# kanyu369/ADNM-UNet

Measured on AMD Instinct MI355X. Metric: sequences/sec training ADNM-UNet 5->20x128x128, higher is better.
Workload: dtype bf16; 1 GPU; ADNM-UNet create_ADNMUNet(5,20,6) 128x128 full training step (fwd + enRainfallLoss + bwd + clip_grad_norm_ + AdamW), recipe parameters, synthetic radar frames in HBM; per_gpu_batch=4, global_batch=4, frames=5->20, parallelism=single, launch=hipGraph replay

## Files before the change

### adnm-unet_amd/csrc/conv3.hip

```cpp
#include "adnm_common.h"

namespace {

using f32x4 = adnm_f32x4;
constexpr int kBlock = 256, kWaves = 4;
constexpr int CK = 16, CKP = CK + 4;
constexpr int MB = 2;
constexpr int kTilePix = kWaves * MB * 16;

struct Geo {
  int TW, RB, TH;
  int tiles_x, tiles_y, VR;
};
inline Geo make_geo(int64_t B, int64_t H, int64_t W) {
  Geo g;
  g.TW = (W == 4 || W == 8) ? (int)W : 16;
  g.RB = 16 / g.TW;
  g.TH = kWaves * MB * g.RB;
  g.VR = (int)(B * (H + 1));
  g.tiles_x = (int)adnm_cdiv(W, g.TW);
  g.tiles_y = (int)adnm_cdiv(g.VR, g.TH);
  return g;
}

// ... 222 lines not shown
  }
  if (rec_a) adnm_amax_commit(&a.q->amax_a, amax_a);
  if (rec_b) adnm_amax_commit(&a.q->amax_b, amax_b);
  if (PREC == ADNM_MFMA_FP8) {
    const float inv = 1.0f / (q_sa * q_sb);
#pragma unroll
    for (int nb = 0; nb < NB; ++nb)
#pragma unroll
      for (int mb = 0; mb < MB; ++mb) acc[nb][mb] = acc[nb][mb] * inv;
  }
  conv3_epilogue<NB, ACT_OUT>(a, acc, wave, kk, dyj, dxj, x0, v0, n0);
}

template <int NB, int ACT_IN, int ACT_OUT>
__global__ __launch_bounds__(kBlock) void conv3_bf16_kernel(ConvArgs a) {
  extern __shared__ __attribute__((aligned(16))) float smem[];
  constexpr int CN = 2 * CK;
  float amax_a = 0.f, amax_b = 0.f;
  bool rec_a = false, rec_b = false;
  if (a.q) {
    const bool rec = a.q->record != 0.f;
    rec_a = rec && blockIdx.y == 0, rec_b = rec && blockIdx.x == 0;
  }
  const int TWp = a.TW + 2;
  float* sIn = smem;
  float* sW = smem + (a.TH + 2) * TWp * CKP;
  const int wave = threadIdx.x >> 6, lane = threadIdx.x & 63, j = lane & 15, kk = lane >> 4;
  const int tx = blockIdx.x % a.tiles_x, ty = blockIdx.x / a.tiles_x;
  const int x0 = tx * a.TW, v0 = ty * a.TH, n0 = blockIdx.y * NB * 16;
  const int dyj = j / a.TW, dxj = j - dyj * a.TW;
  int base[MB];
#pragma unroll
  for (int mb = 0; mb < MB; ++mb) base[mb] = (((wave * MB + mb) * a.RB + dyj) * TWp + dxj) * CKP + 4 * kk;
  f32x4 acc[NB][MB];
#pragma unroll
  for (int nb = 0; nb < NB; ++nb)
#pragma unroll
    for (int mb = 0; mb < MB; ++mb) acc[nb][mb] = f32x4{0.f, 0.f, 0.f, 0.f};
  const int kbeg = blockIdx.z * a.chunks_per_split * CK;
  const int kend = kbeg + a.chunks_per_split * CK < a.K ? kbeg + a.chunks_per_split * CK : a.K;
  constexpr int kItIn = 4;
  constexpr int kItW = (9 * NB * 64 + kBlock - 1) / kBlock;
  const int PT = (a.TH + 2) * TWp;
  float rin[kItIn][8], rw[kItW][8];
  auto load_chunk = [&](int c0) {
#pragma unroll
    for (int u = 0; u < kItIn; ++u) {
      const int it = threadIdx.x + u * kBlock;
      const int pix = it >> 2, q = it & 3, r = pix / TWp, cc = pix - r * TWp, ch = c0 + 8 * q;
      const int64_t p = it < PT * 4 ? pixel_of(v0 - 1 + r, x0 - 1 + cc, a.B, a.H, a.W, a.VR) : -1;
      float v[8] = {0.f, 0.f, 0.f, 0.f, 0.f, 0.f, 0.f, 0.f};
      if (p >= 0 && ch < kend) {
        if (a.vec_in && ch + 7 < kend) {
          const float4 t0 = *reinterpret_cast<const float4*>(a.in + p * a.ldin + ch), t1 = *reinterpret_cast<const float4*>(a.in + p * a.ldin + ch + 4);
          v[0] = t0.x; v[1] = t0.y; v[2] = t0.z; v[3] = t0.w; v[4] = t1.x; v[5] = t1.y; v[6] = t1.z; v[7] = t1.w;
          if (ACT_IN != ADNM_ACT_NONE) {
            const float4 g0 = *reinterpret_cast<const float4*>(a.in2 + p * a.ldin2 + ch), g1 = *reinterpret_cast<const float4*>(a.in2 + p * a.ldin2 + ch + 4);
            v[0] *= act_grad<ACT_IN>(g0.x); v[1] *= act_grad<ACT_IN>(g0.y); v[2] *= act_grad<ACT_IN>(g0.z); v[3] *= act_grad<ACT_IN>(g0.w);
            v[4] *= act_grad<ACT_IN>(g1.x); v[5] *= act_grad<ACT_IN>(g1.y); v[6] *= act_grad<ACT_IN>(g1.z); v[7] *= act_grad<ACT_IN>(g1.w);
          }
        } else {
#pragma unroll
          for (int e = 0; e < 8; ++e)
            if (ch + e < kend) {
              v[e] = a.in[p * a.ldin + ch + e];
              if (ACT_IN != ADNM_ACT_NONE) v[e] *= act_grad<ACT_IN>(a.in2[p * a.ldin2 + ch + e]);
            }
        }
      }
#pragma unroll
      for (int e = 0; e < 8; ++e) rin[u][e] = v[e];
    }
#pragma unroll
    for (int u = 0; u < kItW; ++u) {
      const int it = threadIdx.x + u * kBlock;
      const int kq = it & 3, nl = (it >> 2) % (NB * 16), tap = it / (NB * 64);
      const int n = n0 + nl, k0 = c0 + 8 * kq;
      float v[8] = {0.f, 0.f, 0.f, 0.f, 0.f, 0.f, 0.f, 0.f};
      if (it < 9 * NB * 64 && n < a.N && k0 < kend) {
        const float* wp = a.w + (int64_t)n * a.sn + (int64_t)(a.flip ? 8 - tap : tap) * a.st + (int64_t)k0 * a.sk;
        if (a.vec_w && k0 + 7 < kend) {
          const float4 t0 = *reinterpret_cast<const float4*>(wp), t1 = *reinterpret_cast<const float4*>(wp + 4);
          v[0] = t0.x; v[1] = t0.y; v[2] = t0.z; v[3] = t0.w; v[4] = t1.x; v[5] = t1.y; v[6] = t1.z; v[7] = t1.w;
        } else {
#pragma unroll
          for (int e = 0; e < 8; ++e)
            if (k0 + e < kend) v[e] = wp[(int64_t)e * a.sk];
        }
      }
#pragma unroll
      for (int e = 0; e < 8; ++e) rw[u][e] = v[e];
    }
  };
  auto store_chunk = [&]() {
#pragma unroll
    for (int u = 0; u < kItIn; ++u) {
      const int it = threadIdx.x + u * kBlock;
      if (it >= PT * 4) break;
      if (rec_a) amax_a = adnm_amax4(adnm_amax4(amax_a, rin[u][0], rin[u][1], rin[u][2], rin[u][3]), rin[u][4], rin[u][5], rin[u][6], rin[u][7]);
      *reinterpret_cast<adnm_bf16x8*>(sIn + (it >> 2) * CKP + 4 * (it & 3)) = adnm_pack_bf16x8(rin[u]);
    }
#pragma unroll
    for (int u = 0; u < kItW; ++u) {
      const int it = threadIdx.x + u * kBlock;
      if (it >= 9 * NB * 64) break;
      const int kq = it & 3, nl = (it >> 2) % (NB * 16), tap = it / (NB * 64);
      if (rec_b) amax_b = adnm_amax4(adnm_amax4(amax_b, rw[u][0], rw[u][1], rw[u][2], rw[u][3]), rw[u][4], rw[u][5], rw[u][6], rw[u][7]);
      *reinterpret_cast<adnm_bf16x8*>(sW + (tap * NB * 16 + nl) * CKP + 4 * kq) = adnm_pack_bf16x8(rw[u]);
    }
  };
  if (kbeg < kend) load_chunk(kbeg);
  for (int c0 = kbeg; c0 < kend; c0 += CN) {
    __syncthreads();
    store_chunk();
    __syncthreads();
    if (c0 + CN < kend) load_chunk(c0 + CN);
#pragma unroll
    for (int tap = 0; tap < 9; ++tap) {
      const int toff = ((tap / 3) * TWp + (tap % 3)) * CKP;
      adnm_bf16x8 fw[NB], fx[MB];
#pragma unroll
      for (int nb = 0; nb < NB; ++nb) fw[nb] = *reinterpret_cast<const adnm_bf16x8*>(sW + (tap * NB * 16 + nb * 16 + j) * CKP + 4 * kk);
#pragma unroll
      for (int mb = 0; mb < MB; ++mb) fx[mb] = *reinterpret_cast<const adnm_bf16x8*>(sIn + base[mb] + toff);
#pragma unroll
      for (int nb = 0; nb < NB; ++nb)
#pragma unroll
        for (int mb = 0; mb < MB; ++mb) acc[nb][mb] = __builtin_amdgcn_mfma_f32_16x16x32_bf16(fw[nb], fx[mb], acc[nb][mb], 0, 0, 0);
    }
  }
  if (rec_a) adnm_amax_commit(&a.q->amax_a, amax_a);
  if (rec_b) adnm_amax_commit(&a.q->amax_b, amax_b);
  conv3_epilogue<NB, ACT_OUT>(a, acc, wave, kk, dyj, dxj, x0, v0, n0);
}

template <int ACT_OUT>
__global__ __launch_bounds__(256) void conv3_join_kernel(const float* __restrict__ part, int nsplit, int64_t M, int N, const float* __restrict__ bias,
                                                         float* __restrict__ out, int64_t ldo, float* __restrict__ pre, int64_t ldpre) {
  const int nq = N >> 2;
  const int64_t i = (int64_t)blockIdx.x * 256 + threadIdx.x;
  if (i >= M * nq) return;
  const int64_t p = i / nq;
  const int n = (int)(i - p * nq) * 4;
  float4 s = *reinterpret_cast<const float4*>(part + p * N + n);
  for (int z = 1; z < nsplit; ++z) {
    const float4 t = *reinterpret_cast<const float4*>(part + ((int64_t)z * M + p) * N + n);
    s.x += t.x; s.y += t.y; s.z += t.z; s.w += t.w;
  }
  if (bias) { s.x += bias[n]; s.y += bias[n + 1]; s.z += bias[n + 2]; s.w += bias[n + 3]; }
  if (pre) *reinterpret_cast<float4*>(pre + p * ldpre + n) = s;
  *reinterpret_cast<float4*>(out + p * ldo + n) = make_float4(act_fwd<ACT_OUT>(s.x), act_fwd<ACT_OUT>(s.y), act_fwd<ACT_OUT>(s.z), act_fwd<ACT_OUT>(s.w));
}

struct WgArgs {
  const float* dout; int64_t lddo;
  const float* pre;  int64_t ldpre;
  const float* in;   int64_t ldin;
  float* part; int64_t rowlen;
  int want_bias;
  int B, H, W, K, N, ntiles;
  int TW, RB, TH, VR, tiles_x;
  int vec_in, vec_do;
};

template <int NB, int ACT, int PREC>
__global__ __launch_bounds__(kBlock) void conv3_wgrad_kernel(WgArgs a) {
  constexpr int DP = NB * 16 + 16;
  extern __shared__ __attribute__((aligned(16))) float smem[];
  const int TWp = a.TW + 2;
  float* sIn = smem;
  float* sD = smem + (a.TH + 2) * TWp * CKP;
  const int wave = threadIdx.x >> 6, lane = threadIdx.x & 63, j = lane & 15, kk = lane >> 4;
  const int c0 = blockIdx.y * CK, n0 = blockIdx.z * NB * 16;
  f32x4 acc[9][NB];
#pragma unroll
  for (int t = 0; t < 9; ++t)
#pragma unroll
    for (int nb = 0; nb < NB; ++nb) acc[t][nb] = f32x4{0.f, 0.f, 0.f, 0.f};
  float bsum = 0.f;
  constexpr int kItIn = 4, kItD = (kTilePix * NB * 4 + kBlock - 1) / kBlock;
  const int PT = (a.TH + 2) * TWp;
  float rin[kItIn][4], rd[kItD][4];
  auto load_tile = [&](int tile) {
    const int tx = tile % a.tiles_x, ty = tile / a.tiles_x, x0 = tx * a.TW, v0 = ty * a.TH;
#pragma unroll
    for (int u = 0; u < kItIn; ++u) {
      const int it = threadIdx.x + u * kBlock;
      const int pix = it >> 2, q = it & 3, r = pix / TWp, cc = pix - r * TWp, ch = c0 + 4 * q;
      const int64_t p = it < PT * 4 ? pixel_of(v0 - 1 + r, x0 - 1 + cc, a.B, a.H, a.W, a.VR) : -1;
      float v[4] = {0.f, 0.f, 0.f, 0.f};
      if (p >= 0 && ch < a.K) {
        if (a.vec_in && ch + 3 < a.K) {
          const float4 t = *reinterpret_cast<const float4*>(a.in + p * a.ldin + ch);
          v[0] = t.x; v[1] = t.y; v[2] = t.z; v[3] = t.w;
        } else {
#pragma unroll
          for (int e = 0; e < 4; ++e)
            if (ch + e < a.K) v[e] = a.in[p * a.ldin + ch + e];
        }
      }
#pragma unroll
      for (int e = 0; e < 4; ++e) rin[u][e] = v[e];
    }
#pragma unroll
    for (int u = 0; u < kItD; ++u) {
      const int it = threadIdx.x + u * kBlock;
      const int pxl = it / (NB * 4), q = it - pxl * (NB * 4), n = n0 + 4 * q;
      const int pb = pxl >> 4, jj = pxl & 15, dy_ = jj / a.TW, dx_ = jj - dy_ * a.TW;
      const int64_t p = it < kTilePix * NB * 4 ? pixel_of(v0 + pb * a.RB + dy_, x0 + dx_, a.B, a.H, a.W, a.VR) : -1;
      float v[4] = {0.f, 0.f, 0.f, 0.f};
      if (p >= 0 && n < a.N) {
        if (a.vec_do && n + 3 < a.N) {
          const float4 t = *reinterpret_cast<const float4*>(a.dout + p * a.lddo + n);
          v[0] = t.x; v[1] = t.y; v[2] = t.z; v[3] = t.w;
          if (ACT != ADNM_ACT_NONE) {
            const float4 g = *reinterpret_cast<const float4*>(a.pre + p * a.ldpre + n);
            v[0] *= act_grad<ACT>(g.x); v[1] *= act_grad<ACT>(g.y); v[2] *= act_grad<ACT>(g.z); v[3] *= act_grad<ACT>(g.w);
          }
        } else {
#pragma unroll
          for (int e = 0; e < 4; ++e)
            if (n + e < a.N) {
              v[e] = a.dout[p * a.lddo + n + e];
              if (ACT != ADNM_ACT_NONE) v[e] *= act_grad<ACT>(a.pre[p * a.ldpre + n + e]);
            }
        }
      }
#pragma unroll
      for (int e = 0; e < 4; ++e) rd[u][e] = v[e];
    }
  };
  auto store_tile = [&]() {
#pragma unroll
    for (int u = 0; u < kItIn; ++u) {
      const int it = threadIdx.x + u * kBlock;
      if (it >= PT * 4) break;
      *reinterpret_cast<float4*>(sIn + (it >> 2) * CKP + 4 * (it & 3)) = make_float4(rin[u][0], rin[u][1], rin[u][2], rin[u][3]);
    }
#pragma unroll
    for (int u = 0; u < kItD; ++u) {
      const int it = threadIdx.x + u * kBlock;
      if (it >= kTilePix * NB * 4) break;
      const int pxl = it / (NB * 4), q = it - pxl * (NB * 4);
      *reinterpret_cast<float4*>(sD + pxl * DP + 4 * q) = make_float4(rd[u][0], rd[u][1], rd[u][2], rd[u][3]);
    }
  };
  if ((int)blockIdx.x < a.ntiles) load_tile(blockIdx.x);
  for (int tile = blockIdx.x; tile < a.ntiles; tile += gridDim.x) {
    __syncthreads();
    store_tile();
    __syncthreads();
    if (tile + (int)gridDim.x < a.ntiles) load_tile(tile + gridDim.x);
    static_assert(MB == 2, "the weight-gradient step pairs the wave's two pixel blocks");
    float av[NB][2][4];
    const float* bp[2][4];
#pragma unroll
    for (int pbw = 0; pbw < MB; ++pbw) {
      const int pb = wave * MB + pbw;
#pragma unroll
      for (int e = 0; e < 4; ++e) {
        const int jj = 4 * kk + e, pxl = pb * 16 + jj, dy_ = jj / a.TW, dx_ = jj - dy_ * a.TW;
#pragma unroll
        for (int nb = 0; nb < NB; ++nb) av[nb][pbw][e] = sD[pxl * DP + nb * 16 + j];
        bp[pbw][e] = sIn + ((pb * a.RB + dy_) * TWp + dx_) * CKP + j;
      }
    }
    AdnmFrag<PREC> fa[NB];
#pragma unroll
    for (int nb = 0; nb < NB; ++nb) fa[nb] = adnm_make_frag<PREC, false>(av[nb][0], av[nb][1], 1.f);
#pragma unroll
    for (int tap = 0; tap < 9; ++tap) {
      const int toff = ((tap / 3) * TWp + (tap % 3)) * CKP;
      const float b0[4] = {bp[0][0][toff], bp[0][1][toff], bp[0][2][toff], bp[0][3][toff]};
      const float b1[4] = {bp[1][0][toff], bp[1][1][toff], bp[1][2][toff], bp[1][3][toff]};
      const AdnmFrag<PREC> fb = adnm_make_frag<PREC, false>(b0, b1, 1.f);
#pragma unroll
      for (int nb = 0; nb < NB; ++nb) acc[tap][nb] = adnm_mma<PREC, false, false>(fa[nb], fb, acc[tap][nb]);
    }
    if (a.want_bias && blockIdx.y == 0 && lane < NB * 16) {
#pragma unroll 8
      for (int p = 0; p < MB * 16; ++p) bsum += sD[(wave * MB * 16 + p) * DP + lane];
    }
  }
  __syncthreads();
  float* red = smem;
  constexpr int kPer = 9 * NB * 4;
#pragma unroll
  for (int tap = 0; tap < 9; ++tap)
#pragma unroll
    for (int nb = 0; nb < NB; ++nb)
#pragma unroll
      for (int r = 0; r < 4; ++r) red[(wave * (kPer + 1) + (tap * NB + nb) * 4 + r) * 64 + lane] = acc[tap][nb][r];
  red[(wave * (kPer + 1) + kPer) * 64 + lane] = bsum;
  __syncthreads();
  float* dst = a.part + (int64_t)blockIdx.x * a.rowlen;
  for (int e = threadIdx.x; e < (kPer + 1) * 64; e += kBlock) {
    const float v = (red[e] + red[(kPer + 1) * 64 + e]) + (red[2 * (kPer + 1) * 64 + e] + red[3 * (kPer + 1) * 64 + e]);
    const int slot = e >> 6, ln = e & 63;
    if (slot == kPer) {
      if (a.want_bias && blockIdx.y == 0 && ln < NB * 16 && n0 + ln < a.N) dst[(int64_t)a.N * 9 * a.K + n0 + ln] = v;
      continue;
    }
    const int r = slot & 3, nb = (slot >> 2) % NB, tap = slot / (4 * NB);
    const int n = n0 + nb * 16 + (ln >> 4) * 4 + r, k = c0 + (ln & 15);
    if (n < a.N && k < a.K) dst[((int64_t)n * 9 + tap) * a.K + k] = v;
  }
}

inline bool al16(const void* p) { return ((uintptr_t)p & 15) == 0; }

int check_shape(const char* who, int64_t B, int64_t H, int64_t W, int64_t K, int64_t N) {
  ADNM_REQUIRE(B > 0 && H > 0 && W > 0 && K > 0 && N > 0, "%s: empty shape", who);
  ADNM_REQUIRE(B * (H + 1) < (1ll << 30) && B * H * W < (1ll << 31) && K <= 65536 && N <= 65536, "%s: shape too large", who);
  return ADNM_OK;
}

struct Split {
  int nb, ngroups, nsplit, cps;
};
inline Split plan_split(const Geo& g, int64_t K, int64_t N) {
  Split s;
  s.nb = N > 32 ? 4 : (N > 16 ? 2 : 1);
  s.ngroups = (int)adnm_cdiv(N, s.nb * 16);
  const int nchunks = (int)adnm_cdiv(K, CK);
  const int64_t blocks = (int64_t)g.tiles_x * g.tiles_y * s.ngroups;
  int want = 1;
  if (blocks < 256 && nchunks >= 4 && N % 4 == 0) {
    want = (int)adnm_cdiv(512, blocks);
    if (want > nchunks / 2) want = nchunks / 2;
    if (want > 16) want = 16;
    if (want < 1) want = 1;
  }
  s.cps = (int)adnm_cdiv(nchunks, want);
  if (want > 1 && (s.cps & 1)) ++s.cps;
  s.nsplit = (int)adnm_cdiv(nchunks, s.cps);
  return s;
}

template <int ACT_IN, int ACT_OUT>
int launch_conv(const ConvArgs& a, const Geo& g, const Split& s, int prec, hipStream_t st, const char* prof, double bytes) {
  const size_t smem = sizeof(float) * ((size_t)(g.TH + 2) * (g.TW + 2) * CKP + (size_t)9 * s.nb * 16 * CKP);
  const dim3 grid((unsigned)(g.tiles_x * g.tiles_y), (unsigned)s.ngroups, (unsigned)s.nsplit);
  ADNM_PROF(prof, st, bytes);
#define CV(PRECV, BF8V)                                                                                  \
  do {                                                                                                   \
    if (s.nb == 4) conv3_kernel<4, ACT_IN, ACT_OUT, PRECV, BF8V><<<grid, kBlock, smem, st>>>(a);         \
    else if (s.nb == 2) conv3_kernel<2, ACT_IN, ACT_OUT, PRECV, BF8V><<<grid, kBlock, smem, st>>>(a);    \
    else conv3_kernel<1, ACT_IN, ACT_OUT, PRECV, BF8V><<<grid, kBlock, smem, st>>>(a);                   \
  } while (0)
  static const bool fp32_images = getenv("ADNM_CONV3_FP32_IMAGES") && atoi(getenv("ADNM_CONV3_FP32_IMAGES")) != 0;
  if (prec == ADNM_MFMA_BF16 && fp32_images) CV(ADNM_MFMA_BF16, false);
  else if (prec == ADNM_MFMA_BF16) {
    if (s.nb == 4) conv3_bf16_kernel<4, ACT_IN, ACT_OUT><<<grid, kBlock, smem, st>>>(a);
    else if (s.nb == 2) conv3_bf16_kernel<2, ACT_IN, ACT_OUT><<<grid, kBlock, smem, st>>>(a);
    else conv3_bf16_kernel<1, ACT_IN, ACT_OUT><<<grid, kBlock, smem, st>>>(a);
  } else if (prec == ADNM_MFMA_FP8) CV(ADNM_MFMA_FP8, false);
  else if (prec == ADNM_MFMA_FP8_GRAD) CV(ADNM_MFMA_FP8, true);
  else CV(ADNM_MFMA_F32, false);
#undef CV
  return ADNM_OK;
}

void fill_geo(ConvArgs& a, const Geo& g) { a.TW = g.TW, a.RB = g.RB, a.TH = g.TH, a.VR = g.VR, a.tiles_x = g.tiles_x; }

}

extern "C" int64_t adnm_conv3_ws_bytes(int64_t B, int64_t H, int64_t W, int64_t K, int64_t N) {
  if (B <= 0 || H <= 0 || W <= 0 || K <= 0 || N <= 0) return 0;
  const Geo g = make_geo(B, H, W);
  const Split s = plan_split(g, K, N);
  return s.nsplit > 1 ? (int64_t)s.nsplit * B * H * W * N * (int64_t)sizeof(float) : 16;
}

extern "C" int adnm_conv3_fwd(const float* in, int64_t ldin, const float* w, int64_t ws_n, int64_t ws_tap, int64_t ws_k, const float* bias,
                              float* out, int64_t ldo, float* pre, int64_t ldpre, void* ws, int64_t ws_bytes, int64_t B, int64_t H, int64_t W,
                              int64_t K, int64_t N, int act, int prec, float* q, adnm_stream_t stream) {
  if (int rc = check_shape("conv3_fwd", B, H, W, K, N)) return rc;
  ADNM_REQUIRE(in && w && out, "conv3_fwd: null pointer");
  ADNM_REQUIRE(prec >= ADNM_MFMA_F32 && prec <= ADNM_MFMA_FP8, "conv3_fwd: bad prec %d", prec);
  ADNM_REQUIRE(prec != ADNM_MFMA_FP8 || q, "conv3_fwd: the fp8 mode needs a quantisation record");
  ADNM_REQUIRE(ldin >= K && ldo >= N && (!pre || ldpre >= N), "conv3_fwd: row strides smaller than the rows");
  ADNM_REQUIRE(act == ADNM_ACT_NONE || act == ADNM_ACT_GELU, "conv3_fwd: activation %d not in {none, gelu}", act);
  const Geo g = make_geo(B, H, W);
  const Split s = plan_split(g, K, N);
  if (s.nsplit > 1 && (!ws || ws_bytes < adnm_conv3_ws_bytes(B, H, W, K, N))) {
    adnm_set_error("conv3_fwd: workspace %lld < %lld bytes", (long long)ws_bytes, (long long)adnm_conv3_ws_bytes(B, H, W, K, N));
    return ADNM_EWORKSPACE;
  }
  ConvArgs a{};
  a.in = in, a.ldin = ldin, a.in2 = nullptr, a.ldin2 = 0;
  a.w = w, a.sn = ws_n, a.st = ws_tap, a.sk = ws_k, a.flip = 0;
  a.bias = bias, a.out = out, a.ldo = ldo, a.pre = pre, a.ldpre = ldpre, a.part = (float*)ws;
  a.B = (int)B, a.H = (int)H, a.W = (int)W, a.K = (int)K, a.N = (int)N, a.nsplit = s.nsplit, a.chunks_per_split = s.cps;
  fill_geo(a, g);
  a.vec_in = al16(in) && ldin % 4 == 0 && K % 4 == 0;
  a.vec_w = ws_k == 1 && al16(w) && ws_n % 4 == 0 && ws_tap % 4 == 0 && K % 4 == 0;
  a.vec_out = al16(out) && ldo % 4 == 0 && N % 4 == 0 && (!pre || (al16(pre) && ldpre % 4 == 0));
  a.q = reinterpret_cast<AdnmQuant*>(q);
  hipStream_t st = (hipStream_t)stream;
  const double bytes = 4.0 * ((double)B * H * W * (K + N * (pre ? 2 : 1)) + 9.0 * K * N);
  if (act == ADNM_ACT_GELU && s.nsplit == 1) launch_conv<ADNM_ACT_NONE, ADNM_ACT_GELU>(a, g, s, prec, st, "conv3_fwd", bytes);
  else launch_conv<ADNM_ACT_NONE, ADNM_ACT_NONE>(a, g, s, prec, st, "conv3_fwd", bytes);
  ADNM_CHECK_LAUNCH("conv3_fwd");
  if (s.nsplit > 1) {
    const int64_t M = B * H * W, nthreads = M * (N / 4);
    ADNM_PROF("conv3_join", st, 4.0 * M * N * (s.nsplit + 1 + (pre ? 1 : 0)));
    if (act == ADNM_ACT_GELU)
      conv3_join_kernel<ADNM_ACT_GELU><<<(unsigned)adnm_cdiv(nthreads, 256), 256, 0, st>>>((const float*)ws, s.nsplit, M, (int)N, bias, out, ldo, pre, ldpre);
    else
      conv3_join_kernel<ADNM_ACT_NONE><<<(unsigned)adnm_cdiv(nthreads, 256), 256, 0, st>>>((const float*)ws, s.nsplit, M, (int)N, bias, out, ldo, pre, ldpre);
    ADNM_CHECK_LAUNCH("conv3_join");
  }
  return ADNM_OK;
}

extern "C" int adnm_conv3_dgrad(const float* dout, int64_t lddo, const float* pre, int64_t ldpre, int act, const float* w, int64_t ws_n,
                                int64_t ws_tap, int64_t ws_k, float* din, int64_t lddin, void* ws, int64_t ws_bytes, int64_t B, int64_t H,
                                int64_t W, int64_t K, int64_t N, int prec, float* q, adnm_stream_t stream) {
  if (int rc = check_shape("conv3_dgrad", B, H, W, K, N)) return rc;
  ADNM_REQUIRE(dout && w && din, "conv3_dgrad: null pointer");
  ADNM_REQUIRE(prec >= ADNM_MFMA_F32 && prec <= ADNM_MFMA_FP8_GRAD, "conv3_dgrad: bad prec %d", prec);
  ADNM_REQUIRE((prec != ADNM_MFMA_FP8 && prec != ADNM_MFMA_FP8_GRAD) || q, "conv3_dgrad: the fp8 modes need a quantisation record");
  if (prec == ADNM_MFMA_FP8) prec = ADNM_MFMA_FP8_GRAD;
  ADNM_REQUIRE(act == ADNM_ACT_NONE || (act == ADNM_ACT_GELU && pre), "conv3_dgrad: activation %d needs the saved pre-activation", act);
  ADNM_REQUIRE(lddo >= N && lddin >= K && (!pre || ldpre >= N), "conv3_dgrad: row strides smaller than the rows");
  const Geo g = make_geo(B, H, W);
  const Split s = plan_split(g, N, K);
  if (s.nsplit > 1 && (!ws || ws_bytes < adnm_conv3_ws_bytes(B, H, W, N, K))) {
    adnm_set_error("conv3_dgrad: workspace %lld < %lld bytes", (long long)ws_bytes, (long long)adnm_conv3_ws_bytes(B, H, W, N, K));
    return ADNM_EWORKSPACE;
  }
  ConvArgs a{};
  a.in = dout, a.ldin = lddo, a.in2 = pre, a.ldin2 = ldpre;
  a.w = w, a.sn = ws_k, a.st = ws_tap, a.sk = ws_n, a.flip = 1;
  a.bias = nullptr, a.out = din, a.ldo = lddin, a.pre = nullptr, a.ldpre = 0, a.part = (float*)ws;
  a.B = (int)B, a.H = (int)H, a.W = (int)W, a.K = (int)N, a.N = (int)K, a.nsplit = s.nsplit, a.chunks_per_split = s.cps;
  fill_geo(a, g);
  a.vec_in = al16(dout) && lddo % 4 == 0 && N % 4 == 0 && (!pre || (al16(pre) && ldpre % 4 == 0));
  a.vec_w = a.sk == 1 && al16(w) && a.sn % 4 == 0 && a.st % 4 == 0 && N % 4 == 0;
  a.vec_out = al16(din) && lddin % 4 == 0 && K % 4 == 0;
  a.q = reinterpret_cast<AdnmQuant*>(q);
  hipStream_t st = (hipStream_t)stream;
  const double bytes = 4.0 * ((double)B * H * W * (K + N * (act != ADNM_ACT_NONE ? 2 : 1)) + 9.0 * K * N);
  if (act == ADNM_ACT_GELU) launch_conv<ADNM_ACT_GELU, ADNM_ACT_NONE>(a, g, s, prec, st, "conv3_dgrad", bytes);
  else launch_conv<ADNM_ACT_NONE, ADNM_ACT_NONE>(a, g, s, prec, st, "conv3_dgrad", bytes);
  ADNM_CHECK_LAUNCH("conv3_dgrad");
  if (s.nsplit > 1) {
    const int64_t M = B * H * W, nthreads = M * (K / 4);
    ADNM_PROF("conv3_join", st, 4.0 * M * K * (s.nsplit + 1));
    conv3_join_kernel<ADNM_ACT_NONE><<<(unsigned)adnm_cdiv(nthreads, 256), 256, 0, st>>>((const float*)ws, s.nsplit, M, (int)K, nullptr, din, lddin, nullptr, 0);
    ADNM_CHECK_LAUNCH("conv3_join");
  }
  return ADNM_OK;
}

namespace {
struct WgPlan {
  int nb, cogroups, cichunks, rows;
  int64_t rowlen;
};
inline WgPlan plan_wgrad(const Geo& g, int64_t K, int64_t N, bool bias) {
  WgPlan p;
  p.nb = N > 16 ? 2 : 1;
  p.cogroups = (int)adnm_cdiv(N, p.nb * 16);
  p.cichunks = (int)adnm_cdiv(K, CK);
  p.rowlen = N * 9 * K + (bias ? N : 0);
  const int64_t ntiles = (int64_t)g.tiles_x * g.tiles_y;
  int64_t r = adnm_cdiv(768, (int64_t)p.cichunks * p.cogroups);
  const int64_t by_mem = (int64_t)(8 << 20) / (p.rowlen * 4);
  if (r > by_mem) r = by_mem;
  if (r > ntiles) r = ntiles;
  if (r > 256) r = 256;
  p.rows = (int)(r < 1 ? 1 : r);
  return p;
}
}

extern "C" int64_t adnm_conv3_wgrad_ws_bytes(int64_t B, int64_t H, int64_t W, int64_t K, int64_t N) {
  if (B <= 0 || H <= 0 || W <= 0 || K <= 0 || N <= 0) return 0;
  const WgPlan p = plan_wgrad(make_geo(B, H, W), K, N, true);
  return (int64_t)p.rows * p.rowlen * (int64_t)sizeof(float);
}

extern "C" int adnm_conv3_wgrad(const float* dout, int64_t lddo, const float* pre, int64_t ldpre, int act, const float* in, int64_t ldin,
                                float* dw, float* dbias, void* ws, int64_t ws_bytes, int64_t B, int64_t H, int64_t W, int64_t K, int64_t N,
                                int prec, adnm_stream_t stream) {
  if (prec == ADNM_MFMA_FP8 || prec == ADNM_MFMA_FP8_GRAD) prec = ADNM_MFMA_BF16;
  if (int rc = check_shape("conv3_wgrad", B, H, W, K, N)) return rc;
  ADNM_REQUIRE(dout && in && dw, "conv3_wgrad: null pointer");
  ADNM_REQUIRE(act == ADNM_ACT_NONE || (act == ADNM_ACT_GELU && pre), "conv3_wgrad: activation %d needs the saved pre-activation", act);
  ADNM_REQUIRE(lddo >= N && ldin >= K && (!pre || ldpre >= N), "conv3_wgrad: row strides smaller than the rows");
  ADNM_REQUIRE(N * 9 * K + N < (1ll << 31), "conv3_wgrad: weight too large");
  const Geo g = make_geo(B, H, W);
  const WgPlan p = plan_wgrad(g, K, N, dbias != nullptr);
  if (!ws || ws_bytes < (int64_t)p.rows * p.rowlen * 4) {
    adnm_set_error("conv3_wgrad: workspace %lld < %lld bytes", (long long)ws_bytes, (long long)((int64_t)p.rows * p.rowlen * 4));
    return ADNM_EWORKSPACE;
  }
  WgArgs a{};
  a.dout = dout, a.lddo = lddo, a.pre = pre, a.ldpre = ldpre, a.in = in, a.ldin = ldin;
  a.part = (float*)ws, a.rowlen = p.rowlen, a.want_bias = dbias != nullptr;
  a.B = (int)B, a.H = (int)H, a.W = (int)W, a.K = (int)K, a.N = (int)N, a.ntiles = g.tiles_x * g.tiles_y;
  a.TW = g.TW, a.RB = g.RB, a.TH = g.TH, a.VR = g.VR, a.tiles_x = g.tiles_x;
  a.vec_in = al16(in) && ldin % 4 == 0 && K % 4 == 0;
  a.vec_do = al16(dout) && lddo % 4 == 0 && N % 4 == 0 && (!pre || (al16(pre) && ldpre % 4 == 0));
  hipStream_t st = (hipStream_t)stream;
  size_t smem = sizeof(float) * ((size_t)(g.TH + 2) * (g.TW + 2) * CKP + (size_t)kTilePix * (p.nb * 16 + 16));
  const size_t red = sizeof(float) * (size_t)kWaves * (9 * p.nb * 4 + 1) * 64;
  if (smem < red) smem = red;
  const dim3 grid((unsigned)p.rows, (unsigned)p.cichunks, (unsigned)p.cogroups);
  {
    ADNM_PROF("conv3_wgrad", st, 4.0 * ((double)B * H * W * (K + N * (act != ADNM_ACT_NONE ? 2 : 1)) + 9.0 * K * N));
#define WG1(NBV, ACTV, BFV)                                                                   \
  do {                                                                                        \
    ADNM_ALLOW_LDS((conv3_wgrad_kernel<NBV, ACTV, BFV>), smem, "conv3_wgrad");                \
    conv3_wgrad_kernel<NBV, ACTV, BFV><<<grid, kBlock, smem, st>>>(a);                        \
  } while (0)
#define WG(NBV)                                                                               \
  do {                                                                                        \
    if (act == ADNM_ACT_GELU) { if (prec == ADNM_MFMA_BF16) WG1(NBV, ADNM_ACT_GELU, ADNM_MFMA_BF16); else WG1(NBV, ADNM_ACT_GELU, ADNM_MFMA_F32); } \
    else { if (prec == ADNM_MFMA_BF16) WG1(NBV, ADNM_ACT_NONE, ADNM_MFMA_BF16); else WG1(NBV, ADNM_ACT_NONE, ADNM_MFMA_F32); }                     \
  } while (0)
    if (p.nb == 2) WG(2);
    else WG(1);
#undef WG
#undef WG1
  }
  ADNM_CHECK_LAUNCH("conv3_wgrad");
  adnm_launch_fold("conv3_wgrad_fold", (const float*)ws, p.rows, (int)p.rowlen, {dw, (int)(N * 9 * K)}, {dbias, dbias ? (int)N : 0}, {nullptr, 0},
                   {nullptr, 0}, st);
  ADNM_CHECK_LAUNCH("conv3_wgrad_fold");
  return ADNM_OK;
}
```

Before: 499.4 sequences/s.

## Restructure conv3 weight-gradient kernel into large channel-block tiles with bf16 LDS

Rewrites the 3x3 conv weight-gradient kernel so each workgroup owns a multi-block output-by-input channel tile (up to 64x64), splitting the waves over channel blocks instead of pixel blocks. Operands are staged in LDS pre-transposed, with three x-shifted copies of the input halo stored in bf16 (or fp32), so MFMA fragments load with vector reads. This also removes the cross-wave LDS reduction, since each wave writes its own partials directly. A planner picks block shapes and split counts against a target workgroup count and a workspace cap, both overridable by environment variables. The cost is more register pressure from larger accumulator arrays and extra LDS write traffic for the triplicated halo.

Result: no change. 499.3 sequences/s (-0.0%).

```diff
diff --git a/adnm-unet_amd/csrc/conv3.hip b/adnm-unet_amd/csrc/conv3.hip
--- a/adnm-unet_amd/csrc/conv3.hip
+++ b/adnm-unet_amd/csrc/conv3.hip
@@ -398,6 +398,7 @@
   *reinterpret_cast<float4*>(out + p * ldo + n) = make_float4(act_fwd<ACT_OUT>(s.x), act_fwd<ACT_OUT>(s.y), act_fwd<ACT_OUT>(s.z), act_fwd<ACT_OUT>(s.w));
 }
 
+constexpr int kWgPix = 128;
 struct WgArgs {
   const float* dout; int64_t lddo;
   const float* pre;  int64_t ldpre;
@@ -405,35 +406,69 @@
   float* part; int64_t rowlen;
   int want_bias;
   int B, H, W, K, N, ntiles;
-  int TW, RB, TH, VR, tiles_x;
+  int TW, TH, VR, tiles_x;
+  int rows, ksplits;
   int vec_in, vec_do;
 };
 
-template <int NB, int ACT, int PREC>
+template <int PREC> struct WgLds;
+template <> struct WgLds<ADNM_MFMA_BF16> { using T = uint16_t; static constexpr int PD = 136, IP = 168; };
+template <> struct WgLds<ADNM_MFMA_F32> { using T = float; static constexpr int PD = 132, IP = 164; };
+__device__ __forceinline__ void wg_put(uint16_t* p, float v) { *p = f32_to_bf16(v); }
+__device__ __forceinline__ void wg_put(float* p, float v) { *p = v; }
+__device__ __forceinline__ AdnmFrag<ADNM_MFMA_BF16> wg_frag(const uint16_t* p) {
+  AdnmFrag<ADNM_MFMA_BF16> f;
+  f.v = *reinterpret_cast<const adnm_bf16x8*>(p);
+  return f;
+}
+__device__ __forceinline__ AdnmFrag<ADNM_MFMA_F32> wg_frag(const float* p) {
+  AdnmFrag<ADNM_MFMA_F32> f;
+  const float4 t0 = *reinterpret_cast<const float4*>(p), t1 = *reinterpret_cast<const float4*>(p + 4);
+  f.v[0] = t0.x, f.v[1] = t0.y, f.v[2] = t0.z, f.v[3] = t0.w, f.v[4] = t1.x, f.v[5] = t1.y, f.v[6] = t1.z, f.v[7] = t1.w;
+  return f;
+}
+__device__ __forceinline__ int64_t wg_pixel(int b, int y, int x, int B, int H, int W) {
+  while (y > H) y -= H + 1, ++b;
+  return (y >= 0 && y < H && b < B && x >= 0 && x < W) ? ((int64_t)b * H + y) * W + x : -1;
+}
+constexpr int wg_halo_pixels = 180;
+
+template <int NBO, int NBK, int ACT, int PREC>
 __global__ __launch_bounds__(kBlock) void conv3_wgrad_kernel(WgArgs a) {
-  constexpr int DP = NB * 16 + 16;
+  using T = typename WgLds<PREC>::T;
+  constexpr int PD = WgLds<PREC>::PD, IP = WgLds<PREC>::IP, NO = NBO * 16, KO = NBK * 16, QN = NBO * 4, KQ = NBK * 4;
+  constexpr int WGK = NBK >= 2 ? 2 : 1, WGO = kWaves / WGK, WNO = NBO / WGO, WNK = NBK / WGK;
+  static_assert(NBO % WGO == 0 && NBK % WGK == 0 && QN % 8 == 0, "every wave owns whole (output, input) block pairs");
   extern __shared__ __attribute__((aligned(16))) float smem[];
-  const int TWp = a.TW + 2;
-  float* sIn = smem;
-  float* sD = smem + (a.TH + 2) * TWp * CKP;
+  T* sD = reinterpret_cast<T*>(smem);
+  T* sIn = sD + NO * PD;
+  const int TWp = a.TW + 2, PT = (a.TH + 2) * TWp;
+  const bool wide = a.TW == 16;
+  const int lw = wide ? 4 : 3;
   const int wave = threadIdx.x >> 6, lane = threadIdx.x & 63, j = lane & 15, kk = lane >> 4;
-  const int c0 = blockIdx.y * CK, n0 = blockIdx.z * NB * 16;
-  f32x4 acc[9][NB];
+  const int row = blockIdx.x % a.rows, split = blockIdx.x / a.rows, ks = split % a.ksplits, os = split / a.ksplits;
+  const int n0 = os * NO, c0 = ks * KO, wo = wave / WGK, wk = wave % WGK;
+  const bool do_bias = a.want_bias && ks == 0;
+  f32x4 acc[9][WNO][WNK];
 #pragma unroll
   for (int t = 0; t < 9; ++t)
 #pragma unroll
-    for (int nb = 0; nb < NB; ++nb) acc[t][nb] = f32x4{0.f, 0.f, 0.f, 0.f};
-  float bsum = 0.f;
-  constexpr int kItIn = 4, kItD = (kTilePix * NB * 4 + kBlock - 1) / kBlock;
-  const int PT = (a.TH + 2) * TWp;
-  float rin[kItIn][4], rd[kItD][4];
+    for (int i = 0; i < WNO; ++i)
+#pragma unroll
+      for (int m = 0; m < WNK; ++m) acc[t][i][m] = f32x4{0.f, 0.f, 0.f, 0.f};
+  float bsum[4] = {0.f, 0.f, 0.f, 0.f};
+  constexpr int kItIn = 12 * 16 * KQ / kBlock, kItD = kWgPix * QN / kBlock;
+  static_assert(12 * 16 >= wg_halo_pixels, "item count covers the halo tile");
+  float rin[kItIn][4], rdo[kItD][4], rpr[ACT != ADNM_ACT_NONE ? kItD : 1][4];
   auto load_tile = [&](int tile) {
     const int tx = tile % a.tiles_x, ty = tile / a.tiles_x, x0 = tx * a.TW, v0 = ty * a.TH;
+    const int b0 = v0 > 0 ? (v0 - 1) / (a.H + 1) : 0, y0 = v0 - 1 - b0 * (a.H + 1);
 #pragma unroll
     for (int u = 0; u < kItIn; ++u) {
-      const int it = threadIdx.x + u * kBlock;
-      const int pix = it >> 2, q = it & 3, r = pix / TWp, cc = pix - r * TWp, ch = c0 + 4 * q;
-      const int64_t p = it < PT * 4 ? pixel_of(v0 - 1 + r, x0 - 1 + cc, a.B, a.H, a.W, a.VR) : -1;
+      const int it = threadIdx.x + u * kBlock, rest = it >> 6;
+      const int kq = (rest % (KQ / 4)) * 4 + (it & 3), hp = (rest / (KQ / 4)) * 16 + ((it >> 2) & 15);
+      const int r = wide ? hp / 18 : hp / 10, c = hp - r * TWp, ch = c0 + 4 * kq;
+      const int64_t p = hp < PT ? wg_pixel(b0, y0 + r, x0 - 1 + c, a.B, a.H, a.W) : -1;
       float v[4] = {0.f, 0.f, 0.f, 0.f};
       if (p >= 0 && ch < a.K) {
         if (a.vec_in && ch + 3 < a.K) {
@@ -450,106 +485,109 @@
     }
 #pragma unroll
     for (int u = 0; u < kItD; ++u) {
-      const int it = threadIdx.x + u * kBlock;
-      const int pxl = it / (NB * 4), q = it - pxl * (NB * 4), n = n0 + 4 * q;
-      const int pb = pxl >> 4, jj = pxl & 15, dy_ = jj / a.TW, dx_ = jj - dy_ * a.TW;
-      const int64_t p = it < kTilePix * NB * 4 ? pixel_of(v0 + pb * a.RB + dy_, x0 + dx_, a.B, a.H, a.W, a.VR) : -1;
-      float v[4] = {0.f, 0.f, 0.f, 0.f};
+      const int it = threadIdx.x + u * kBlock, rest = it >> 6;
+      const int q = (rest % (QN / 4)) * 4 + (it & 3), pxl = (rest / (QN / 4)) * 16 + ((it >> 2) & 15);
+      const int pr = pxl >> lw, pc = pxl & (a.TW - 1), n = n0 + 4 * q;
+      const int64_t p = wg_pixel(b0, y0 + 1 + pr, x0 + pc, a.B, a.H, a.W);
+      float v[4] = {0.f, 0.f, 0.f, 0.f}, g[4] = {0.f, 0.f, 0.f, 0.f};
       if (p >= 0 && n < a.N) {
         if (a.vec_do && n + 3 < a.N) {
           const float4 t = *reinterpret_cast<const float4*>(a.dout + p * a.lddo + n);
           v[0] = t.x; v[1] = t.y; v[2] = t.z; v[3] = t.w;
           if (ACT != ADNM_ACT_NONE) {
-            const float4 g = *reinterpret_cast<const float4*>(a.pre + p * a.ldpre + n);
-            v[0] *= act_grad<ACT>(g.x); v[1] *= act_grad<ACT>(g.y); v[2] *= act_grad<ACT>(g.z); v[3] *= act_grad<ACT>(g.w);
+            const float4 s = *reinterpret_cast<const float4*>(a.pre + p * a.ldpre + n);
+            g[0] = s.x; g[1] = s.y; g[2] = s.z; g[3] = s.w;
           }
         } else {
 #pragma unroll
           for (int e = 0; e < 4; ++e)
             if (n + e < a.N) {
               v[e] = a.dout[p * a.lddo + n + e];
-              if (ACT != ADNM_ACT_NONE) v[e] *= act_grad<ACT>(a.pre[p * a.ldpre + n + e]);
+              if (ACT != ADNM_ACT_NONE) g[e] = a.pre[p * a.ldpre + n + e];
             }
         }
       }
 #pragma unroll
-      for (int e = 0; e < 4; ++e) rd[u][e] = v[e];
+      for (int e = 0; e < 4; ++e) {
+        rdo[u][e] = v[e];
+        if (ACT != ADNM_ACT_NONE) rpr[u][e] = g[e];
+      }
     }
   };
   auto store_tile = [&]() {
 #pragma unroll
     for (int u = 0; u < kItIn; ++u) {
-      const int it = threadIdx.x + u * kBlock;
-      if (it >= PT * 4) break;
-      *reinterpret_cast<float4*>(sIn + (it >> 2) * CKP + 4 * (it & 3)) = make_float4(rin[u][0], rin[u][1], rin[u][2], rin[u][3]);
+      const int it = threadIdx.x + u * kBlock, rest = it >> 6;
+      const int kq = (rest % (KQ / 4)) * 4 + (it & 3), hp = (rest / (KQ / 4)) * 16 + ((it >> 2) & 15);
+      if (hp >= PT) continue;
+      const int r = wide ? hp / 18 : hp / 10, c = hp - r * TWp;
+#pragma unroll
+      for (int tx = 0; tx < 3; ++tx) {
+        const int x = c - tx;
+        if (x < 0 || x >= a.TW) continue;
+#pragma unroll
+        for (int e = 0; e < 4; ++e) wg_put(sIn + (tx * KO + 4 * kq + e) * IP + r * a.TW + x, rin[u][e]);
+      }
     }
 #pragma unroll
     for (int u = 0; u < kItD; ++u) {
-      const int it = threadIdx.x + u * kBlock;
-      if (it >= kTilePix * NB * 4) break;
-      const int pxl = it / (NB * 4), q = it - pxl * (NB * 4);
-      *reinterpret_cast<float4*>(sD + pxl * DP + 4 * q) = make_float4(rd[u][0], rd[u][1], rd[u][2], rd[u][3]);
+      const int it = threadIdx.x + u * kBlock, rest = it >> 6;
+      const int q = (rest % (QN / 4)) * 4 + (it & 3), pxl = (rest / (QN / 4)) * 16 + ((it >> 2) & 15);
+#pragma unroll
+      for (int e = 0; e < 4; ++e) {
+        const float v = ACT != ADNM_ACT_NONE ? rdo[u][e] * act_grad<ACT>(rpr[u][e]) : rdo[u][e];
+        bsum[e] += v;
+        wg_put(sD + (4 * q + e) * PD + pxl, v);
+      }
     }
   };
-  if ((int)blockIdx.x < a.ntiles) load_tile(blockIdx.x);
-  for (int tile = blockIdx.x; tile < a.ntiles; tile += gridDim.x) {
+  if (row < a.ntiles) load_tile(row);
+  for (int tile = row; tile < a.ntiles; tile += a.rows) {
     __syncthreads();
     store_tile();
     __syncthreads();
-    if (tile + (int)gridDim.x < a.ntiles) load_tile(tile + gridDim.x);
-    static_assert(MB == 2, "the weight-gradient step pairs the wave's two pixel blocks");
-    float av[NB][2][4];
-    const float* bp[2][4];
-#pragma unroll
-    for (int pbw = 0; pbw < MB; ++pbw) {
-      const int pb = wave * MB + pbw;
-#pragma unroll
-      for (int e = 0; e < 4; ++e) {
-        const int jj = 4 * kk + e, pxl = pb * 16 + jj, dy_ = jj / a.TW, dx_ = jj - dy_ * a.TW;
-#pragma unroll
-        for (int nb = 0; nb < NB; ++nb) av[nb][pbw][e] = sD[pxl * DP + nb * 16 + j];
-        bp[pbw][e] = sIn + ((pb * a.RB + dy_) * TWp + dx_) * CKP + j;
-      }
-    }
-    AdnmFrag<PREC> fa[NB];
-#pragma unroll
-    for (int nb = 0; nb < NB; ++nb) fa[nb] = adnm_make_frag<PREC, false>(av[nb][0], av[nb][1], 1.f);
-#pragma unroll
-    for (int tap = 0; tap < 9; ++tap) {
-      const int toff = ((tap / 3) * TWp + (tap % 3)) * CKP;
-      const float b0[4] = {bp[0][0][toff], bp[0][1][toff], bp[0][2][toff], bp[0][3][toff]};
-      const float b1[4] = {bp[1][0][toff], bp[1][1][toff], bp[1][2][toff], bp[1][3][toff]};
-      const AdnmFrag<PREC> fb = adnm_make_frag<PREC, false>(b0, b1, 1.f);
-#pragma unroll
-      for (int nb = 0; nb < NB; ++nb) acc[tap][nb] = adnm_mma<PREC, false, false>(fa[nb], fb, acc[tap][nb]);
-    }
-    if (a.want_bias && blockIdx.y == 0 && lane < NB * 16) {
-#pragma unroll 8
-      for (int p = 0; p < MB * 16; ++p) bsum += sD[(wave * MB * 16 + p) * DP + lane];
-    }
-  }
-  __syncthreads();
-  float* red = smem;
-  constexpr int kPer = 9 * NB * 4;
+    if (tile + a.rows < a.ntiles) load_tile(tile + a.rows);
+#pragma unroll
+    for (int g = 0; g < kWgPix / 32; ++g) {
+      AdnmFrag<PREC> fa[WNO];
+#pragma unroll
+      for (int i = 0; i < WNO; ++i) fa[i] = wg_frag(sD + ((wo * WNO + i) * 16 + j) * PD + g * 32 + kk * 8);
+#pragma unroll
+      for (int tap = 0; tap < 9; ++tap) {
+        AdnmFrag<PREC> fb[WNK];
+#pragma unroll
+        for (int m = 0; m < WNK; ++m)
+          fb[m] = wg_frag(sIn + ((tap % 3) * KO + (wk * WNK + m) * 16 + j) * IP + g * 32 + kk * 8 + (tap / 3) * a.TW);
+#pragma unroll
+        for (int i = 0; i < WNO; ++i)
+#pragma unroll
+          for (int m = 0; m < WNK; ++m) acc[tap][i][m] = adnm_mma<PREC, false, false>(fa[i], fb[m], acc[tap][i][m]);
+      }
+    }
+  }
+  float* dst = a.part + (int64_t)row * a.rowlen;
 #pragma unroll
   for (int tap = 0; tap < 9; ++tap)
 #pragma unroll
-    for (int nb = 0; nb < NB; ++nb)
-#pragma unroll
-      for (int r = 0; r < 4; ++r) red[(wave * (kPer + 1) + (tap * NB + nb) * 4 + r) * 64 + lane] = acc[tap][nb][r];
-  red[(wave * (kPer + 1) + kPer) * 64 + lane] = bsum;
-  __syncthreads();
-  float* dst = a.part + (int64_t)blockIdx.x * a.rowlen;
-  for (int e = threadIdx.x; e < (kPer + 1) * 64; e += kBlock) {
-    const float v = (red[e] + red[(kPer + 1) * 64 + e]) + (red[2 * (kPer + 1) * 64 + e] + red[3 * (kPer + 1) * 64 + e]);
-    const int slot = e >> 6, ln = e & 63;
-    if (slot == kPer) {
-      if (a.want_bias && blockIdx.y == 0 && ln < NB * 16 && n0 + ln < a.N) dst[(int64_t)a.N * 9 * a.K + n0 + ln] = v;
-      continue;
-    }
-    const int r = slot & 3, nb = (slot >> 2) % NB, tap = slot / (4 * NB);
-    const int n = n0 + nb * 16 + (ln >> 4) * 4 + r, k = c0 + (ln & 15);
-    if (n < a.N && k < a.K) dst[((int64_t)n * 9 + tap) * a.K + k] = v;
+    for (int i = 0; i < WNO; ++i)
+#pragma unroll
+      for (int m = 0; m < WNK; ++m)
+#pragma unroll
+        for (int r = 0; r < 4; ++r) {
+          const int n = n0 + (wo * WNO + i) * 16 + kk * 4 + r, k = c0 + (wk * WNK + m) * 16 + j;
+          if (n < a.N && k < a.K) dst[((int64_t)n * 9 + tap) * a.K + k] = acc[tap][i][m][r];
+        }
+  if (do_bias) {
+    __syncthreads();
+    smem[threadIdx.x * 4 + 0] = bsum[0], smem[threadIdx.x * 4 + 1] = bsum[1], smem[threadIdx.x * 4 + 2] = bsum[2], smem[threadIdx.x * 4 + 3] = bsum[3];
+    __syncthreads();
+    if (threadIdx.x < NO && n0 + (int)threadIdx.x < a.N) {
+      const int q = threadIdx.x >> 2, e = threadIdx.x & 3;
+      float s = 0.f;
+      for (int w = (q >> 2); w < kWaves; w += QN / 4)
+        for (int pl = 0; pl < 16; ++pl) s += smem[(w * 64 + pl * 4 + (q & 3)) * 4 + e];
+      dst[(int64_t)a.N * 9 * a.K + n0 + threadIdx.x] = s;
+    }
   }
 }
 
@@ -701,30 +739,74 @@
 }
 
 namespace {
+inline Geo make_wgeo(int64_t B, int64_t H, int64_t W) {
+  Geo g = make_geo(B, H, W);
+  if (g.TW == 4) {
+    g.TW = 16, g.RB = 1, g.TH = kWaves * MB;
+    g.tiles_x = 1, g.tiles_y = (int)adnm_cdiv(g.VR, g.TH);
+  }
+  return g;
+}
 struct WgPlan {
-  int nb, cogroups, cichunks, rows;
+  int nbo, nbk, osplits, ksplits, rows;
   int64_t rowlen;
 };
-inline WgPlan plan_wgrad(const Geo& g, int64_t K, int64_t N, bool bias) {
+inline int env_int(const char* name, int dflt) {
+  const char* v = getenv(name);
+  return v && *v ? atoi(v) : dflt;
+}
+inline WgPlan plan_wgrad(const Geo& g, int64_t K, int64_t N, bool bias, int prec) {
   WgPlan p;
-  p.nb = N > 16 ? 2 : 1;
-  p.cogroups = (int)adnm_cdiv(N, p.nb * 16);
-  p.cichunks = (int)adnm_cdiv(K, CK);
   p.rowlen = N * 9 * K + (bias ? N : 0);
   const int64_t ntiles = (int64_t)g.tiles_x * g.tiles_y;
-  int64_t r = adnm_cdiv(768, (int64_t)p.cichunks * p.cogroups);
-  const int64_t by_mem = (int64_t)(8 << 20) / (p.rowlen * 4);
-  if (r > by_mem) r = by_mem;
+  static const int cap_mb = env_int("ADNM_WG_CAP_MB", 16), target = env_int("ADNM_WG_TARGET", 256), force = env_int("ADNM_WG_FORCE", 0);
+  int64_t r = ((int64_t)cap_mb << 20) / ((N * 9 * K + N) * 4);
   if (r > ntiles) r = ntiles;
   if (r > 256) r = 256;
+  if (r >= 8) r &= ~(int64_t)7;
   p.rows = (int)(r < 1 ? 1 : r);
+  static const int cand[5][2] = {{4, 4}, {4, 2}, {2, 4}, {2, 2}, {4, 1}};
+  const int nbk_max = K > 32 ? 4 : (K > 16 ? 2 : 1), nbo_max = N > 32 ? 4 : 2;
+  p.nbo = 0;
+  for (int c = 0; c < 5; ++c) {
+    const int nbo = cand[c][0], nbk = cand[c][1];
+    if (force ? force != nbo * 10 + nbk : false) continue;
+    if (!force) {
+      if (nbk_max == 1 ? nbk != 1 : (nbk == 1 || nbk > nbk_max)) continue;
+      if (nbk != 1 && nbo > nbo_max) continue;
+    }
+    if (prec != ADNM_MFMA_BF16 && nbk == 4) continue;
+    p.nbo = nbo, p.nbk = nbk;
+    p.osplits = (int)adnm_cdiv(N, nbo * 16), p.ksplits = (int)adnm_cdiv(K, nbk * 16);
+    if ((int64_t)p.rows * p.osplits * p.ksplits >= target) break;
+  }
   return p;
+}
+template <int NBO, int NBK, int ACT, int PREC>
+int launch_wgrad(const WgArgs& a, unsigned grid, hipStream_t st) {
+  using L = WgLds<PREC>;
+  const size_t smem = sizeof(typename L::T) * ((size_t)NBO * 16 * L::PD + (size_t)3 * NBK * 16 * L::IP);
+  ADNM_ALLOW_LDS((conv3_wgrad_kernel<NBO, NBK, ACT, PREC>), smem, "conv3_wgrad");
+  conv3_wgrad_kernel<NBO, NBK, ACT, PREC><<<grid, kBlock, smem, st>>>(a);
+  return ADNM_OK;
+}
+template <int ACT, int PREC>
+int launch_wgrad_blocks(const WgPlan& p, const WgArgs& a, unsigned grid, hipStream_t st) {
+  if (p.nbo == 4 && p.nbk == 2) return launch_wgrad<4, 2, ACT, PREC>(a, grid, st);
+  if (p.nbo == 2 && p.nbk == 2) return launch_wgrad<2, 2, ACT, PREC>(a, grid, st);
+  if (p.nbo == 4 && p.nbk == 1) return launch_wgrad<4, 1, ACT, PREC>(a, grid, st);
+  if constexpr (PREC == ADNM_MFMA_BF16) {
+    if (p.nbo == 4 && p.nbk == 4) return launch_wgrad<4, 4, ACT, PREC>(a, grid, st);
+    if (p.nbo == 2 && p.nbk == 4) return launch_wgrad<2, 4, ACT, PREC>(a, grid, st);
+  }
+  adnm_set_error("conv3_wgrad: no kernel for the %d x %d channel block", p.nbo * 16, p.nbk * 16);
+  return ADNM_EINVAL;
 }
 }
 
 extern "C" int64_t adnm_conv3_wgrad_ws_bytes(int64_t B, int64_t H, int64_t W, int64_t K, int64_t N) {
   if (B <= 0 || H <= 0 || W <= 0 || K <= 0 || N <= 0) return 0;
-  const WgPlan p = plan_wgrad(make_geo(B, H, W), K, N, true);
+  const WgPlan p = plan_wgrad(make_wgeo(B, H, W), K, N, true, ADNM_MFMA_BF16);
   return (int64_t)p.rows * p.rowlen * (int64_t)sizeof(float);
 }
 
@@ -734,11 +816,12 @@
   if (prec == ADNM_MFMA_FP8 || prec == ADNM_MFMA_FP8_GRAD) prec = ADNM_MFMA_BF16;
   if (int rc = check_shape("conv3_wgrad", B, H, W, K, N)) return rc;
   ADNM_REQUIRE(dout && in && dw, "conv3_wgrad: null pointer");
+  ADNM_REQUIRE(prec == ADNM_MFMA_F32 || prec == ADNM_MFMA_BF16, "conv3_wgrad: bad prec %d", prec);
   ADNM_REQUIRE(act == ADNM_ACT_NONE || (act == ADNM_ACT_GELU && pre), "conv3_wgrad: activation %d needs the saved pre-activation", act);
   ADNM_REQUIRE(lddo >= N && ldin >= K && (!pre || ldpre >= N), "conv3_wgrad: row strides smaller than the rows");
   ADNM_REQUIRE(N * 9 * K + N < (1ll << 31), "conv3_wgrad: weight too large");
-  const Geo g = make_geo(B, H, W);
-  const WgPlan p = plan_wgrad(g, K, N, dbias != nullptr);
+  const Geo g = make_wgeo(B, H, W);
+  const WgPlan p = plan_wgrad(g, K, N, dbias != nullptr, prec);
   if (!ws || ws_bytes < (int64_t)p.rows * p.rowlen * 4) {
     adnm_set_error("conv3_wgrad: workspace %lld < %lld bytes", (long long)ws_bytes, (long long)((int64_t)p.rows * p.rowlen * 4));
     return ADNM_EWORKSPACE;
@@ -747,30 +830,18 @@
   a.dout = dout, a.lddo = lddo, a.pre = pre, a.ldpre = ldpre, a.in = in, a.ldin = ldin;
   a.part = (float*)ws, a.rowlen = p.rowlen, a.want_bias = dbias != nullptr;
   a.B = (int)B, a.H = (int)H, a.W = (int)W, a.K = (int)K, a.N = (int)N, a.ntiles = g.tiles_x * g.tiles_y;
-  a.TW = g.TW, a.RB = g.RB, a.TH = g.TH, a.VR = g.VR, a.tiles_x = g.tiles_x;
+  a.TW = g.TW, a.TH = g.TH, a.VR = g.VR, a.tiles_x = g.tiles_x;
+  a.rows = p.rows, a.ksplits = p.ksplits;
   a.vec_in = al16(in) && ldin % 4 == 0 && K % 4 == 0;
   a.vec_do = al16(dout) && lddo % 4 == 0 && N % 4 == 0 && (!pre || (al16(pre) && ldpre % 4 == 0));
   hipStream_t st = (hipStream_t)stream;
-  size_t smem = sizeof(float) * ((size_t)(g.TH + 2) * (g.TW + 2) * CKP + (size_t)kTilePix * (p.nb * 16 + 16));
-  const size_t red = sizeof(float) * (size_t)kWaves * (9 * p.nb * 4 + 1) * 64;
-  if (smem < red) smem = red;
-  const dim3 grid((unsigned)p.rows, (unsigned)p.cichunks, (unsigned)p.cogroups);
+  const unsigned grid = (unsigned)(p.rows * p.osplits * p.ksplits);
   {
     ADNM_PROF("conv3_wgrad", st, 4.0 * ((double)B * H * W * (K + N * (act != ADNM_ACT_NONE ? 2 : 1)) + 9.0 * K * N));
-#define WG1(NBV, ACTV, BFV)                                                                   \
-  do {                                                                                        \
-    ADNM_ALLOW_LDS((conv3_wgrad_kernel<NBV, ACTV, BFV>), smem, "conv3_wgrad");                \
-    conv3_wgrad_kernel<NBV, ACTV, BFV><<<grid, kBlock, smem, st>>>(a);                        \
-  } while (0)
-#define WG(NBV)                                                                               \
-  do {                                                                                        \
-    if (act == ADNM_ACT_GELU) { if (prec == ADNM_MFMA_BF16) WG1(NBV, ADNM_ACT_GELU, ADNM_MFMA_BF16); else WG1(NBV, ADNM_ACT_GELU, ADNM_MFMA_F32); } \
-    else { if (prec == ADNM_MFMA_BF16) WG1(NBV, ADNM_ACT_NONE, ADNM_MFMA_BF16); else WG1(NBV, ADNM_ACT_NONE, ADNM_MFMA_F32); }                     \
-  } while (0)
-    if (p.nb == 2) WG(2);
-    else WG(1);
-#undef WG
-#undef WG1
+    int rc;
+    if (act == ADNM_ACT_GELU) rc = prec == ADNM_MFMA_BF16 ? launch_wgrad_blocks<ADNM_ACT_GELU, ADNM_MFMA_BF16>(p, a, grid, st) : launch_wgrad_blocks<ADNM_ACT_GELU, ADNM_MFMA_F32>(p, a, grid, st);
+    else rc = prec == ADNM_MFMA_BF16 ? launch_wgrad_blocks<ADNM_ACT_NONE, ADNM_MFMA_BF16>(p, a, grid, st) : launch_wgrad_blocks<ADNM_ACT_NONE, ADNM_MFMA_F32>(p, a, grid, st);
+    if (rc) return rc;
   }
   ADNM_CHECK_LAUNCH("conv3_wgrad");
   adnm_launch_fold("conv3_wgrad_fold", (const float*)ws, p.rows, (int)p.rowlen, {dw, (int)(N * 9 * K)}, {dbias, dbias ? (int)N : 0}, {nullptr, 0},
```
